# quadram-institute-bioscience/tatajuba

Measured on AMD Instinct MI355X. Metric: reads/s (whole node), 150 bp synthetic FASTQ, homopolymer scan + context histogram, higher is better.
Workload: dtype u8/u64

## Files before the change

### tatajuba_amd/csrc/hopo_device.hip

```cpp

#include <hip/hip_runtime.h>
#include <rccl/rccl.h>
#include <dlfcn.h>
#include <mutex>
#include <string>
#include <new>
#include <stdint.h>
#include <stdio.h>
#include <stdlib.h>
#include <string.h>
#include <stdarg.h>
#include <limits.h>
#include <float.h>
#include <algorithm>
#include <vector>

#include "../../include/tatajuba_amd.h"
#include "../../include/tatajuba_variants.h"
#include "../../include/tatajuba_features.h"
#include "../../include/tatajuba_effects.h"
#include "../../include/tatajuba_locate.h"

typedef unsigned long long u64;
typedef unsigned int u32;
// ... 1544 lines not shown
        }
      }
      else
      for (int cb0 = 0; cb0 < ncand; cb0 += FK_BLOCK) {
        if (!all_fit) sink.reserve1 ((u32) min (ncand - cb0, FK_BLOCK));
        if (cb0 + 64 * wave >= ncand) continue;
        const int ci = cb0 + tid;
        const bool valid = ci < ncand;
        const u32 s = T.cand[min (ci, ncand - 1)];
        const u32 q = s + 1u, u = s - vk;
        const u32 *ps = &T.st[q >> 5], *pl = &T.lt[u >> 5], *pc = &T.code[u >> 4];
        u32 s0 = ps[0], s1 = ps[1], l0 = pl[0], l1 = pl[1], w0 = pc[0], w1 = pc[1], w2 = pc[2];
        asm volatile ("" : "+v"(s0), "+v"(s1), "+v"(l0), "+v"(l1), "+v"(w0), "+v"(w1), "+v"(w2));
        const u32 len = (u32) __builtin_ctz (__builtin_amdgcn_alignbit (s1, s0, q) | 0x80000000u) + 1u;
        const u32 need = len + vk2;
        const u32 room = v32 - need;
        const u32 notl = ~__builtin_amdgcn_alignbit (l1, l0, u);
        const u32 bad = __builtin_amdgcn_bitop3_b32 (notl << (room & 31u), room >> 31, (len - (valid ? vmp : 0x1000u)) >> 31, 0xFE);
        const bool ok = bad == 0u;
        if (valid && (int) room < 0) {
          const u64 rec = fast_general_tract (T, seq, n_bytes, tile * (long) FK_OWN - FK_HL, (int) s, k, mprime, (ncand_all >= 0x40000000u));
          if (rec != 0ull) sink.store1 (atomicAdd (&sink.L.n, 1u), (u32) rec, (u32) (rec >> 32));
        }
        const u64 okm = __builtin_amdgcn_ballot_w64 (ok);
        u32 araw;
        lds_add_issue (sink.count_addr (), (u32) __builtin_popcountll (okm), araw);
        const u32 sh = u + u;
        const u32 clo = __builtin_amdgcn_alignbit (w1, w0, sh), chi = __builtin_amdgcn_alignbit (w2, w1, sh);
        const u32 l = clo & vkm;
        const u32 cb = (clo >> vk2) & 3u;
        const u32 r = (u32) ((((u64) chi << 32) | clo) >> (vk2 + len + len)) & vkm;
        u32 rcl = revcomp_v32 (l, M55, vrs), rcr = revcomp_v32 (r, M55, vrs);
        if ((ncand_all >= 0x40000000u)) {
          const u32 nb = bits32 (T.np, (int) u);
          if ((nb << ((v32 - need) & 31u)) != 0u && need <= 32u) {
            rcl = revcomp_v32 (l | (u32) spread_pairs (nb & ((1u << k) - 1u)), M55, vrs);
            rcr = revcomp_v32 (r | (u32) spread_pairs ((nb >> ((u32) k + len)) & ((1u << k) - 1u)), M55, vrs);
          }
        }
        const bool rev = cb >= 2u;
        const u32 c0 = rev ? rcr : l, c1 = rev ? rcl : r;
        const u32 fld24 = __builtin_amdgcn_perm (0u, 0x10140C08u, (cb << 24) | 0x000C0C0Cu);
        const u32 lo = c1 | (len << 24);
        const u32 hi = c0 | fld24;
        const u32 at = lds_collect (araw) + (u32) __builtin_amdgcn_mbcnt_hi ((u32) (okm >> 32), __builtin_amdgcn_mbcnt_lo ((u32) okm, 0u));
        if constexpr (LOG) sink.store1ok (ok, at, lo, hi, (u32) lane);
        else sink.store1v (ok ? at : (u32) sink.S + (u32) lane, lo, hi, vh0, vh1, vm27);
      }
    }
    lds_barrier ();
    if (nt >= grp_end) { gpar ^= 1u; grp_end = nt + FK_GROUP; }
    tile = nt;
    it++;
  }
  flush_slow ();
  sink.finish ();
}

#define PL_BLOCK 512
#define PL_WG_PER_CU 2
template <int W>
__global__ __launch_bounds__ (PL_BLOCK, PL_BLOCK * PL_WG_PER_CU / 256)
void partition_log_kernel (LogSpace LG, Buckets BK, DevCounters *ctr, int k)
{
  static_assert (W == 1 || W == 2, "the log holds one-word and two-word records");
  typedef StageLds<W, 2> Lds;
  __shared__ Lds L;
  constexpr u32 RB = TJ_LOGB / W;
  static_assert (Lds::S == (int) RB && Lds::WS == W, "one pass per log block");
  constexpr u32 RR = RB / PL_BLOCK;
  static_assert (RR % 4 == 0, "bins are kept four to a register");
  const u32 tid = threadIdx.x, lane = tid & 63u;
  const u32 wave = (u32) __builtin_amdgcn_readfirstlane ((int) (tid >> 6));
  if (tid < TJ_P) L.hist[tid] = 0;
  u32 cur_j = TJ_EMPTY, cur_chunk = TJ_NOCHUNK;
  lds_barrier ();
  const u32 n_blocks = min (*LG.next, LG.n_blocks);
  u32 b = blockIdx.x;
  if (b >= n_blocks) return;
  u64 w[RR][W];
  u32 n = min (LG.count[b], RB), nn = 0;
  auto load_block = [&] (u32 blk, u32 cnt) {
    const u64 *__restrict__ src = LG.log + ((u64) blk << TJ_LOGB_SHIFT);
    const u32 w0 = tid & ~63u;
#pragma unroll
    for (u32 r = 0; r < RR; r++) {
#pragma unroll
      for (int j = 0; j < W; j++) w[r][j] = 0;
      if (w0 + r * PL_BLOCK < cnt) {
        if constexpr (W == 1) w[r][0] = (src + r * PL_BLOCK)[tid];
        else { const ulonglong2 v = reinterpret_cast<const ulonglong2 *> (src + 2u * r * PL_BLOCK)[tid]; w[r][0] = v.x; w[r][1] = v.y; }
      }
    }
  };
  auto bucket_of = [&] (const u64 *rec) -> u32 {
    if constexpr (W == 1) return bucket_of_rec1 ((u32) rec[0], (u32) (rec[0] >> 32));
    else { u64 c0, c1; u32 base, len10, flag; unpack_raw<W> (rec, k, c0, c1, base, len10, flag); return bucket_of_key (c0, c1, base, len10); }
  };
  load_block (b, n);
  while (true) {
    const u32 bn = b + gridDim.x;
    const bool more = bn < n_blocks;
    if (more) nn = min (LG.count[bn], RB);
    u32 tq = tid;
    asm volatile ("" : "+v"(tq));
    u32 pk[RR / 4];
#pragma unroll
    for (u32 r = 0; r < RR / 4; r++) pk[r] = 0;
    if (n) {
#pragma unroll
      for (u32 r = 0; r < RR; r++) {
        const u32 bin = bucket_of (w[r]);
        pk[r >> 2] |= bin << (8u * (r & 3u));
        if (tid + r * PL_BLOCK < n) atomicAdd (&L.hist[bin], 1u);
      }
      lds_barrier ();
      if (wave < TJ_P / 64) {
        const uint4 h4 = *reinterpret_cast<const uint4 *> (&L.hist[4 * lane]);
        const u32 tot = h4.x + h4.y + h4.z + h4.w;
        const u32 e0 = wave_inclusive_scan (tot) - tot;
        if ((lane >> 4) == wave) *reinterpret_cast<uint4 *> (&L.offs[4 * lane]) = make_uint4 (e0, e0 + h4.x, e0 + h4.x + h4.y, e0 + h4.x + h4.y + h4.z);
        const u32 cnt = L.hist[tid], off = L.offs[tid];
        u64 a1 = 0, a2 = 0;
        u32 thr = off + cnt;
        if (cnt) {
          const u32 p0 = atomicAdd (&BK.cursors[tid * TJ_CSTRIDE], cnt);
          const u32 ch = (u32) TJ_CH0 << BK.ch_shift;
          bucket_claim_ahead_range (BK, tid, p0, cnt, ctr);
          const u32 j0 = chunk_of_pos (BK, p0), j1 = chunk_of_pos (BK, p0 + cnt - 1);
          if (j0 != cur_j) { cur_j = j0; cur_chunk = bucket_chunk_id (BK, tid, j0, true, ctr); }
          if (cur_chunk != TJ_NOCHUNK) a1 = (u64) (size_t) (BK.pool + ((u64) cur_chunk * ch + (p0 - j0 * ch)) * W) - (8ull * W) * off;
          if (j1 != j0) {
            thr = off + ((j0 + 1u) * ch - p0);
            cur_j = j0 + 1u; cur_chunk = bucket_chunk_id (BK, tid, j0 + 1u, true, ctr);
            if (cur_chunk != TJ_NOCHUNK) a2 = (u64) (size_t) (BK.pool + ((u64) cur_chunk * ch) * W) - (8ull * W) * thr;
          }
        }
        reinterpret_cast<uint4 *> (L.gbase)[tid] = make_uint4 ((u32) a1, (u32) (a1 >> 32) | (thr << 16), (u32) a2, (u32) (a2 >> 32));
      }
      lds_barrier ();
      if (tid < TJ_P) L.hist[tid] = 0;
#pragma unroll
      for (u32 r = 0; r < RR; r++)
        if (tid + r * PL_BLOCK < n) {
          const u32 bin = (pk[r >> 2] >> (8u * (r & 3u))) & 255u;
          const u32 d = atomicAdd (&L.offs[bin], 1u);
#pragma unroll
          for (int j = 0; j < W; j++) L.rec[d * W + j] = w[r][j];
          L.bin[d] = (unsigned char) bin;
        }
      lds_barrier ();
      for (u32 r0 = 0; r0 < RR; r0 += 4) {
        if (r0 * PL_BLOCK >= n) break;
        u32 cb[4]; uint4 e[4]; u64 cw[4][W];
#pragma unroll
        for (u32 h = 0; h < 4; h++) cb[h] = L.bin[tq + (r0 + h) * PL_BLOCK];
#pragma unroll
        for (u32 h = 0; h < 4; h++) {
          e[h] = reinterpret_cast<const uint4 *> (L.gbase)[cb[h]];
#pragma unroll
          for (int j = 0; j < W; j++) cw[h][j] = L.rec[(tq + (r0 + h) * PL_BLOCK) * W + j];
        }
#pragma unroll
        for (u32 h = 0; h < 4; h++) {
          const u32 i = tq + (r0 + h) * PL_BLOCK;
          const u64 a = (i < (e[h].y >> 16)) ? (((u64) (e[h].y & 0xFFFFu) << 32) | e[h].x) : (((u64) e[h].w << 32) | e[h].z);
          if (i < n && a != 0ull) {
            typedef __attribute__((address_space(1))) u64 *gwords_t;
            gwords_t q = (gwords_t) (a + (u64) (8u * W * i));
#pragma unroll
            for (int j = 0; j < W; j++) q[j] = cw[h][j];
          }
        }
      }
      lds_barrier ();
    }
    if (!more) break;
    load_block (bn, nn);
    n = nn; b = bn;
  }
}

template <int W>
__global__ void nrun_fixup_bins_kernel (const uint8_t *__restrict__ seq, long n_bytes, int k, int mprime,
                                        Buckets BK, DevCounters *ctr, const FixEntry *fix, u32 fix_cap, int par)
{
  nrun_fixup_entries<W> (seq, n_bytes, k, mprime, BK, ctr, fix, fix_cap, par, blockIdx.x * (u64) blockDim.x + threadIdx.x, (u64) gridDim.x * blockDim.x);
}

template <int W>
__global__ void bin_elems_kernel (const u64 *__restrict__ elems5, long n, int k, Buckets BK, DevCounters *ctr)
{
  for (long i = blockIdx.x * (long) blockDim.x + threadIdx.x; i < n; i += (long) gridDim.x * blockDim.x) {
    const u64 m = elems5[5 * i + 2];
    bucket_insert_slow<W> (elems5[5 * i], elems5[5 * i + 1], (u32) (m & 3ull), (u32) ((m >> TJ_META_LEN_SHIFT) & 0x3FFull),
                           (u32) ((m >> TJ_META_FLAG_SHIFT) & 3ull), k, BK, ctr);
  }
}

template <int W>
__global__ void unpack_buckets_kernel (Buckets BK, int k, u64 *__restrict__ out, u64 cap, u64 *n_out)
{
  const u32 b = blockIdx.x;
  const u32 n = BK.cursors[b * TJ_CSTRIDE];
  for (u32 i = threadIdx.x; i < n; i += blockDim.x) {
    u64 c0, c1; u32 base, len10, flag;
    const u64 at = bucket_slot (BK, b, i, false, nullptr);
    if (at == ~0ull) continue;
    unpack_raw<W> (BK.pool + at * W, k, c0, c1, base, len10, flag);
    if (flag == 3u) continue;
    const u64 o = atomicAdd (n_out, 1ull);
    if (o < cap) { u64 *q = out + 3 * o; q[0] = c0; q[1] = c1; q[2] = make_meta (base, len10, flag); }
  }
}

__global__ void init_table_kernel (u32 *table, u32 maxj, u32 *pool_next)
{
  const u32 b = blockIdx.x * blockDim.x + threadIdx.x;
  if (b < TJ_P) table[(u64) b * maxj] = b;
  if (b == 0) *pool_next = TJ_P;
}

__global__ void clear_buckets_kernel (u32 *cursors, DevCounters *ctr, u32 *table, u32 maxj, int ch_shift, FinCounts *fin, u32 *bins, int nbins,
                                      DevCounters *snap_ctr, u32 *snap_cursors, FinPlan *plan, u32 *__restrict__ fine = nullptr, int fine_bits = 0)
{
  const u32 b = blockIdx.x;
  if (snap_ctr) {
    if (threadIdx.x == 0) {
      snap_cursors[b] = cursors[b * TJ_CSTRIDE];
      if (b == 0) {
        snap_cursors[TJ_P] = cursors[TJ_P * TJ_CSTRIDE];
        if (plan) { plan->n1_exact = (long) fin->n_kept; plan->ovf_exact = fin->overflow; }
      }
    }
    if (b == 0) for (u32 i = threadIdx.x; i < sizeof (DevCounters) / 4; i += blockDim.x) reinterpret_cast<u32 *> (snap_ctr)[i] = reinterpret_cast<const u32 *> (ctr)[i];
    __syncthreads ();
  }
  if (b == 0) for (u32 i = threadIdx.x; i < sizeof (DevCounters) / 4; i += blockDim.x) if (i != offsetof (DevCounters, n_undefined) / 4 && i != offsetof (DevCounters, n_undefined) / 4 + 1) reinterpret_cast<u32 *> (ctr)[i] = 0;
  if (table) {
    u32 used = maxj;
    if (ch_shift >= 0) used = min (maxj, ((cursors[b * TJ_CSTRIDE] / TJ_CH0) >> ch_shift) + 3u);
    for (u32 j = threadIdx.x; j < used; j += blockDim.x) table[(u64) b * maxj + j] = j ? TJ_EMPTY : b;
  }
  if (fine) {
    const int gid = (int) (b * blockDim.x + threadIdx.x), gsz = (int) (gridDim.x * blockDim.x);
    if (plan->ok) {
      const int shift = fine_bits - plan->nbits, run = 1 << shift, nb = plan->nbins;
      for (int i = gid; i < nb; i += gsz) {
        u32 sum = 0;
        if (shift >= 2) {
          uint4 *f4 = reinterpret_cast<uint4 *> (fine) + (size_t) i * (run >> 2);
          for (int j = 0; j < (run >> 2); j++) { const uint4 v = f4[j]; sum += v.x + v.y + v.z + v.w; }
          for (int j = 0; j < (run >> 2); j++) f4[j] = make_uint4 (0, 0, 0, 0);
        }
        else {
          for (int j = 0; j < run; j++) sum += fine[(i << shift) + j];
          for (int j = 0; j < run; j++) fine[(i << shift) + j] = 0;
        }
        bins[i] = sum;
      }
    }
    else for (int i = gid; i < (1 << fine_bits); i += gsz) fine[i] = 0;
// ... 1372 lines not shown
    const u32 st = binstart[bin], s = binstart[bin + 1] - st, o0 = binout[bin];
    for (u32 t0 = 0; t0 < s; t0 += 64) {
      const u32 t = t0 + lane;
      if (t < s) {
        const long u = (long) o0 + tpos[st + t];
        if (u < cap) {
          const u64 a0 = rec[3 * (u64) (st + t)], a1 = rec[3 * (u64) (st + t) + 1], am = rec[3 * (u64) (st + t) + 2];
          const u32 tot = ttot[st + t];
          if (tot != 0xFFFFFFFFu) {
            for (int q = 0; q < n_samples; q++) counts[u * n_samples + q] = 0;
            u64 m = am & ((1ull << TJ_META_SAMPLE_SHIFT) - 1ull);
            m = (m & ~(0xFFFFFull << TJ_META_COUNT_SHIFT)) | (((u64) tot & 0xFFFFFull) << TJ_META_COUNT_SHIFT);
            m = (m & ~(7ull << TJ_META_FLAG_SHIFT)) | ((u64) ((tot >> 28) & 7u) << TJ_META_FLAG_SHIFT);
            keys[3 * u] = a0; keys[3 * u + 1] = a1; keys[3 * u + 2] = m;
          }
        }
      }
      __builtin_amdgcn_wave_barrier ();
      asm volatile ("s_waitcnt vmcnt(0)" ::: "memory");
      if (t < s) {
        const long u = (long) o0 + tpos[st + t];
        if (u < cap) {
          const u64 am = rec[3 * (u64) (st + t) + 2];
          counts[u * n_samples + (int) (am >> TJ_META_SAMPLE_SHIFT)] = meta_count (am);
        }
      }
    }
  }
}

__global__ void set_int_kernel (int *p, int v) { *p = v; }


__global__ void merge_tag_kernel (const u64 *__restrict__ in, u64 *__restrict__ out, long n, const long *__restrict__ starts, int n_samples)
{
  for (long i = blockIdx.x * (long) blockDim.x + threadIdx.x; i < n; i += (long) gridDim.x * blockDim.x) {
    int lo = 0, hi = n_samples;
    while (hi - lo > 1) { const int mid = (lo + hi) >> 1; if (starts[mid] <= i) lo = mid; else hi = mid; }
    out[3 * i] = in[3 * i]; out[3 * i + 1] = in[3 * i + 1];
    out[3 * i + 2] = (in[3 * i + 2] & ((1ull << TJ_META_SAMPLE_SHIFT) - 1ull)) | ((u64) lo << TJ_META_SAMPLE_SHIFT);
  }
}

__global__ void merge_write_kernel (const u64 *__restrict__ rec, long n, const u32 *__restrict__ flags, const u32 *__restrict__ segid,
                                    int n_samples, u64 *__restrict__ keys, int *__restrict__ counts, u32 *__restrict__ totals, u32 *__restrict__ orflags, long cap)
{
  for (long i = blockIdx.x * (long) blockDim.x + threadIdx.x; i < n; i += (long) gridDim.x * blockDim.x) {
    const u32 seg = segid[i] + flags[i] - 1u;
    if ((long) seg >= cap) continue;
    const u64 meta = rec[3 * i + 2];
    const int sample = (int) (meta >> TJ_META_SAMPLE_SHIFT);
    const int cnt = meta_count (meta);
    counts[(long) seg * n_samples + sample] = cnt;
    atomicAdd (&totals[seg], (u32) cnt);
    atomicOr (&orflags[seg], (u32) (meta >> TJ_META_FLAG_SHIFT) & 7u);
    if (flags[i]) { keys[3 * (long) seg] = rec[3 * i]; keys[3 * (long) seg + 1] = rec[3 * i + 1]; keys[3 * (long) seg + 2] = meta; }
  }
}

__global__ void merge_totals_kernel (u64 *__restrict__ keys, const u32 *__restrict__ totals, const u32 *__restrict__ orflags, const u32 *n_seg_p, long cap)
{
  const long n_seg = min ((long) *n_seg_p, cap);
  for (long j = blockIdx.x * (long) blockDim.x + threadIdx.x; j < n_seg; j += (long) gridDim.x * blockDim.x) {
    u64 m = keys[3 * j + 2] & ((1ull << TJ_META_SAMPLE_SHIFT) - 1ull);
    m = (m & ~(0xFFFFFull << TJ_META_COUNT_SHIFT)) | (((u64) totals[j] & 0xFFFFFull) << TJ_META_COUNT_SHIFT);
    m = (m & ~(7ull << TJ_META_FLAG_SHIFT)) | ((u64) (orflags[j] & 7u) << TJ_META_FLAG_SHIFT);
    keys[3 * j + 2] = m;
  }
}



struct DevBuf
{
  void *p = nullptr;
  size_t cap = 0;
};

#define TJ_SCAN_PIECE_TARGET (1ull << 30)

struct DevState { alignas (256) DevCounters ctr; alignas (256) FinCounts fin; alignas (256) u32 cursors[TJ_P + 1]; alignas (256) FinPlan plan;
                  alignas (256) DevCounters snap_ctr; alignas (256) u32 snap_cursors[TJ_P + 1]; alignas (256) u32 pad[4]; };

struct StageTimer
{
  hipEvent_t e0 = nullptr, e1 = nullptr;
  bool timed = false;
  hipError_t create () { const hipError_t e = hipEventCreate (&e0); return e != hipSuccess ? e : hipEventCreate (&e1); }
  void destroy () { if (e0) (void) hipEventDestroy (e0); if (e1) (void) hipEventDestroy (e1); }
  hipError_t begin (hipStream_t stream) { return hipEventRecord (e0, stream); }
  hipError_t end (hipStream_t stream) { return hipEventRecord (e1, stream); }
  bool elapsed (int device, float &ms) const
  { return timed && hipSetDevice (device) == hipSuccess && hipEventSynchronize (e1) == hipSuccess && hipEventElapsedTime (&ms, e0, e1) == hipSuccess; }
  double ms (int device) const { float f = 0.f; return elapsed (device, f) ? (double) f : -1.0; }
};
enum { T_SCAN, T_FIN, T_MERGE, T_TRACT, T_UNION, T_UNION_STATS, T_REF, T_LOCATE, T_LOCATED_TRACTS, T_VARIANTS, T_ANNOTATION, T_TRACT_FEATURES, T_SEED_ORDER, T_LOCATE_GAPPED, T_CODING, T_VARIANT_EFFECTS, TJ_N_TIMERS };

struct tjamd_counter
{
  int device = 0, k = 0, W = 4, n_cu = 256;
  hipStream_t own_stream = nullptr, stream = nullptr;
  DevCounters *d_ctr = nullptr, *h_ctr = nullptr;
  DevCounters *d_lctr = nullptr;
  u32 *d_cursors = nullptr, *h_cursors = nullptr;
  DevBuf pool, table, stage, fix, loc, prefix, rawlist, slow;
  DevBuf log, logmeta;
  int log_mode = 1;
  bool log_next_clean[2] = {false, false};
  hipEvent_t ev_p1 = nullptr;
#define TJ_PIECE_EVENTS 64
  hipEvent_t ev_pa[TJ_PIECE_EVENTS] = {}, ev_pb[TJ_PIECE_EVENTS] = {};
  int n_piece_ev = 0;
  StageTimer timer[TJ_N_TIMERS];
  DevBuf ts_cov, ts_aux;
  long union_cand = -1;
  DevBuf ut_tot, ut_lev, ut_fb, ut_slots;
  DevBuf lc_work;
  bool part_timed = false;
  int fast_mode = 1;
  u32 pool_chunks = 0, maxj = 0;
  int ch_shift = -1;
  u64 bucket_bound = 0;
  u64 chunk_bound = 0;
  long n_raw_known = 0;
  u64 raw_bound = 0;
  long n_undefined = 0;
  double slack = 1.0;
  DevBuf alt, hist, flags, segid, headpos, keep, outpos, scan_tmp, kept, idx_i, idx_f, cov, bins, binstart, binctx, ovf, grp_jt, grp_hist, fine;
  u32 bin_rank_max = BS_RANK_MAX;
  FinCounts *d_fin = nullptr, *h_fin = nullptr;
  struct DevState *d_state = nullptr, *h_state = nullptr;
  void *h_kept = nullptr; size_t h_kept_cap = 0;
  bool bins_zeroed = false;
  bool fine_dirty = false;
  bool bins_counted = false;
  long n_kept = 0; int n_idx = 0, coverage = 0, status = -1;
  hipEvent_t ev_done = nullptr;
  hipEvent_t ev_agg = nullptr;
  hipStream_t order_stream = nullptr;
  int fin_pending = 0;
  int fin_rb = 0, fin_mc = 0; bool fin_speculative = false, fin_plan_ahead = false; u64 fin_kept_cap = 0;
  hipEvent_t marks[8] = {nullptr, nullptr, nullptr, nullptr, nullptr, nullptr, nullptr, nullptr};
  unsigned mark_seq = 0;
  long last_scan_launches = 0;
  unsigned scan_seq = 0;
  size_t piece_target = TJ_SCAN_PIECE_TARGET;
  int scan_grid_cap = 0;
  bool buckets_clean = false;
  long plan_mismatches = 0;
  bool ctr_clean = false;
};

static int ensure (DevBuf &b, size_t bytes, hipStream_t stream, size_t keep_bytes = 0)
{
  if (bytes <= b.cap) return TJAMD_OK;
  size_t want = std::max (bytes, b.cap + b.cap / 2);
  void *np = nullptr;
  hipError_t e = hipMalloc (&np, want);
  if (e != hipSuccess && want > bytes) { want = bytes; e = hipMalloc (&np, want); }
  if (e != hipSuccess) return set_err (TJAMD_ERR_HIP, "hipMalloc of %zu bytes failed: %s", want, hipGetErrorString (e));
  if (b.p) {
    if (keep_bytes) HIPCHK (hipMemcpyAsync (np, b.p, keep_bytes, hipMemcpyDeviceToDevice, stream));
    HIPCHK (hipStreamSynchronize (stream));
    HIPCHK (hipFree (b.p));
  }
  b.p = np; b.cap = want;
  return TJAMD_OK;
}

static void release (DevBuf &b) { if (b.p) (void) hipFree (b.p); b.p = nullptr; b.cap = 0; }

extern "C" tjamd_counter *tjamd_counter_create (int device, int kmer_size)
{
  int n = tjamd_device_count ();
  if (n <= 0) { set_err (TJAMD_ERR_NO_DEVICE, "no HIP device visible: the homopolymer-tract engine needs an MI355X (no CPU fallback)"); return NULL; }
  if (device < 0 || device >= n) { set_err (TJAMD_ERR_ARG, "device %d out of range [0,%d)", device, n); return NULL; }
  if (kmer_size < 2 || kmer_size > 32) { set_err (TJAMD_ERR_ARG, "kmer_size %d outside [2,32] (reference clamp: src/main.c:184-185)", kmer_size); return NULL; }
  HIPCHK_NULL (hipSetDevice (device));
  tjamd_counter *c = new tjamd_counter ();
  c->device = device; c->k = kmer_size;
  c->W = (kmer_size <= 12) ? 1 : (kmer_size <= 28) ? 2 : 4;
  hipDeviceProp_t prop;
  HIPCHK_NULL (hipGetDeviceProperties (&prop, device));
  c->n_cu = prop.multiProcessorCount > 0 ? prop.multiProcessorCount : 256;
  const char *bm = getenv ("TATAJUBA_AMD_BIN_MAX");
  if (bm && atoi (bm) >= 1 && atoi (bm) <= BS_RANK_MAX) c->bin_rank_max = (u32) atoi (bm);
  const char *pc = getenv ("TATAJUBA_AMD_SCAN_PIECE");
  if (pc && atol (pc) >= 4096) c->piece_target = (size_t) atol (pc);
  const char *sk = getenv ("TATAJUBA_AMD_SINK");
  if (sk && !strcmp (sk, "fused")) c->log_mode = 0;
  if (sk && !strcmp (sk, "log")) c->log_mode = 2;
  const char *fm = getenv ("TATAJUBA_AMD_FAST");
  if (fm && atoi (fm) >= 0 && atoi (fm) <= 2) c->fast_mode = atoi (fm);
  const char *sg = getenv ("TATAJUBA_AMD_SCAN_GRID");
  if (sg && atoi (sg) >= 1) c->scan_grid_cap = atoi (sg);
  const char *sl = getenv ("TATAJUBA_AMD_BUCKET_SLACK");
  if (sl && atof (sl) >= 1.0) c->slack = atof (sl);
  HIPCHK_NULL (hipStreamCreateWithFlags (&c->own_stream, hipStreamNonBlocking));
  c->stream = c->own_stream;
  HIPCHK_NULL (hipMalloc ((void **) &c->d_state, sizeof (DevState)));
  HIPCHK_NULL (hipMalloc ((void **) &c->d_lctr, sizeof (DevCounters)));
  HIPCHK_NULL (hipHostMalloc ((void **) &c->h_state, sizeof (DevState), hipHostMallocDefault));
  c->d_ctr = &c->d_state->ctr; c->d_fin = &c->d_state->fin;
  HIPCHK_NULL (hipMalloc ((void **) &c->d_cursors, (size_t) (TJ_P + 1) * TJ_CSTRIDE * 4));
  HIPCHK_NULL (hipMemsetAsync (c->d_cursors, 0, (size_t) (TJ_P + 1) * TJ_CSTRIDE * 4, c->stream));
  c->h_ctr = &c->h_state->ctr; c->h_fin = &c->h_state->fin; c->h_cursors = c->h_state->cursors;
  memset (c->h_state, 0, sizeof (DevState));
  HIPCHK_NULL (hipMemsetAsync (c->d_state, 0, sizeof (DevState), c->stream));
  HIPCHK_NULL (hipMemsetAsync (c->d_lctr, 0, sizeof (DevCounters), c->stream));
  for (StageTimer &t : c->timer) HIPCHK_NULL (t.create ());
  HIPCHK_NULL (hipEventCreate (&c->ev_p1));
  HIPCHK_NULL (hipEventCreateWithFlags (&c->ev_done, hipEventDisableTiming));
  HIPCHK_NULL (hipEventCreateWithFlags (&c->ev_agg, hipEventDisableTiming));
  HIPCHK_NULL (hipStreamSynchronize (c->stream));
  return c;
}

extern "C" void tjamd_counter_destroy (tjamd_counter *c)
{
  if (!c) return;
  (void) hipSetDevice (c->device);
  (void) hipStreamSynchronize (c->stream);
  DevBuf *all[] = {&c->log, &c->logmeta, &c->pool, &c->table, &c->stage, &c->fix, &c->loc, &c->prefix, &c->rawlist, &c->slow, &c->alt, &c->hist, &c->flags, &c->segid, &c->headpos,
                   &c->keep, &c->outpos, &c->scan_tmp, &c->kept, &c->idx_i, &c->idx_f, &c->cov, &c->bins, &c->binstart, &c->binctx, &c->ovf, &c->grp_jt, &c->grp_hist, &c->fine,
                   &c->ts_cov, &c->ts_aux, &c->ut_tot, &c->ut_lev, &c->ut_fb, &c->ut_slots, &c->lc_work};
  for (DevBuf *b : all) release (*b);
  for (hipEvent_t ev : c->marks) if (ev) (void) hipEventDestroy (ev);
  if (c->d_state) (void) hipFree (c->d_state);
  if (c->d_lctr) (void) hipFree (c->d_lctr);
  if (c->d_cursors) (void) hipFree (c->d_cursors);
  if (c->h_state) (void) hipHostFree (c->h_state);
  if (c->h_kept) (void) hipHostFree (c->h_kept);
  for (StageTimer &t : c->timer) t.destroy ();
  if (c->ev_p1) (void) hipEventDestroy (c->ev_p1);
  for (int i = 0; i < TJ_PIECE_EVENTS; i++) { if (c->ev_pa[i]) (void) hipEventDestroy (c->ev_pa[i]); if (c->ev_pb[i]) (void) hipEventDestroy (c->ev_pb[i]); }
  if (c->ev_done) (void) hipEventDestroy (c->ev_done);
  if (c->ev_agg) (void) hipEventDestroy (c->ev_agg);
  if (c->own_stream) (void) hipStreamDestroy (c->own_stream);
  delete c;
}

extern "C" int tjamd_counter_device (const tjamd_counter *c) { return c ? c->device : -1; }

extern "C" int tjamd_counter_set_stream (tjamd_counter *c, void *hip_stream)
{
  if (!c) return set_err (TJAMD_ERR_ARG, "null counter");
  HIPCHK (hipSetDevice (c->device));
  HIPCHK (hipStreamSynchronize (c->stream));
  c->stream = hip_stream ? (hipStream_t) hip_stream : c->own_stream;
  return TJAMD_OK;
}

extern "C" int tjamd_counter_set_order_stream (tjamd_counter *c, void *hip_stream)
{
  if (!c) return set_err (TJAMD_ERR_ARG, "null counter");
  HIPCHK (hipSetDevice (c->device));
  HIPCHK (hipStreamSynchronize (c->stream));
  if (c->order_stream) HIPCHK (hipStreamSynchronize (c->order_stream));
  c->order_stream = (hipStream_t) hip_stream;
  return TJAMD_OK;
}

static Buckets make_buckets (const tjamd_counter *c)
{
  Buckets B;
  B.pool = (u64 *) c->pool.p; B.table = (u32 *) c->table.p; B.cursors = c->d_cursors; B.pool_next = c->d_cursors + TJ_P * TJ_CSTRIDE;
  B.pool_chunks = c->pool_chunks; B.maxj = c->maxj; B.ch_shift = (u32) std::max (c->ch_shift, 0);
  return B;
}

static int clear_buckets (tjamd_counter *c, bool snapshot = false)
{
  if (!c->buckets_clean || snapshot) {
    const bool fused = snapshot && c->fine_dirty && c->bins.p != nullptr;
    hipLaunchKernelGGL (clear_buckets_kernel, dim3 (TJ_P), dim3 (256), 0, c->stream, c->d_cursors, c->d_ctr,
                        (u32 *) (c->maxj ? c->table.p : nullptr), c->maxj, c->ch_shift, c->d_fin, (u32 *) c->bins.p, c->bins.p ? BS_MAXBINS : 0,
                        snapshot ? &c->d_state->snap_ctr : (DevCounters *) nullptr, snapshot ? c->d_state->snap_cursors : (u32 *) nullptr,
                        snapshot ? &c->d_state->plan : (FinPlan *) nullptr, fused ? (u32 *) c->fine.p : (u32 *) nullptr, fine_bin_bits (c->k));
    HIPCHK (hipGetLastError ());
    c->buckets_clean = true;
    c->ctr_clean = true;
    c->bins_zeroed = c->bins.p != nullptr && !fused;
    if (fused) { c->fine_dirty = false; c->bins_counted = true; }
  }
  c->n_raw_known = 0; c->raw_bound = 0; c->bucket_bound = 0; c->chunk_bound = TJ_P; c->ch_shift = -1;
  return TJAMD_OK;
}

extern "C" int tjamd_counter_reset (tjamd_counter *c)
{
  if (!c) return set_err (TJAMD_ERR_ARG, "null counter");
  HIPCHK (hipSetDevice (c->device));
  if (!(c->ctr_clean && c->fin_pending == 0 && c->n_undefined == 0)) HIPCHK (hipMemsetAsync (c->d_ctr, 0, sizeof (DevCounters), c->stream));
  int rc = clear_buckets (c);
// ... 174 lines not shown
  const size_t keep = std::min<size_t> (c->pool.cap, (size_t) (c->chunk_bound * ch * c->W * 8));
  rc = ensure (c->pool, (size_t) ((records / ch + 2 * TJ_P + 1) * ch * c->W * 8), c->stream, keep);
  if (rc) return rc;
  c->pool_chunks = (u32) std::min<u64> (c->pool.cap / (ch * c->W * 8), TJ_NOCHUNK - 1);
  c->buckets_clean = c->buckets_clean && c->table.p != nullptr;
  return ensure_table (c, (c->bucket_bound + records + ch - 1) / ch + 3);
}

static int scan_device_piece (tjamd_counter *c, const void *d_stream, size_t n_bytes, int min_tract_size, bool first, bool last)
{
  int rc = TJAMD_OK;
  if (n_bytes < 64 && d_stream != c->stage.p) {
    rc = ensure (c->stage, 256, c->stream);
    if (rc) return rc;
    HIPCHK (hipMemcpyAsync (c->stage.p, d_stream, n_bytes, hipMemcpyDeviceToDevice, c->stream));
    d_stream = c->stage.p;
  }
  const int mprime = std::max (min_tract_size, 2);
  const u64 bound = (u64) ((double) (n_bytes / (size_t) mprime + 1) * c->slack);
  const long n_tiles = (long) ((n_bytes + TJ_SB_TILE - 1) / TJ_SB_TILE);
  const int grid = (int) std::min<long> (n_tiles, (long) c->n_cu * TJ_SB_WG_PER_CU);
  rc = ensure_buckets (c, bound, grid + 1);
  c->raw_bound += (u64) (n_bytes / (size_t) mprime) + 1u;
  if (!rc) rc = ensure (c->fix, (size_t) TJ_FIX_CAP * sizeof (FixEntry), c->stream);
  const long n_ftiles = (long) ((n_bytes + FK_OWN - 1) / FK_OWN);
  const int fgrid = (int) std::min<long> (n_ftiles, (long) c->n_cu * FK_WG_PER_CU);
  const int lgrid = (int) std::min<long> (n_ftiles * ((FK_OWN + TJ_SB_TILE - 1) / TJ_SB_TILE), (long) c->n_cu * TJ_SB_WG_PER_CU);
  if (!rc && c->fast_mode) rc = ensure (c->slow, (size_t) n_ftiles * 4 + 64, c->stream);
  if (rc) return rc;
  const uint8_t *seq = (const uint8_t *) d_stream;
  const Buckets BK = make_buckets (c);
  FixEntry *fix = (FixEntry *) c->fix.p;
  const int par = (int) (c->scan_seq++ & 1u);
  if (first) HIPCHK (c->timer[T_SCAN].begin (c->stream));
  const TileSrc plain = {nullptr, 0};
  auto capped = [c] (long g) { return (unsigned) (c->scan_grid_cap >= 1 ? std::min<long> (g, (long) c->scan_grid_cap) : g); };
  const bool use_fast = c->fast_mode && n_bytes < ((size_t) 1 << 31) - (1u << 20);
  const bool use_log = use_fast && c->W <= c->log_mode;
  LogSpace LG = {nullptr, nullptr, nullptr, 0u};
  const int fgrid_log = (int) std::min<long> (n_ftiles, (long) c->n_cu * FK_LOG_WG_PER_CU);
  if (use_log) {
    const u64 n_blocks = ((bound * (u64) c->W) >> TJ_LOGB_SHIFT) + 3ull * (u64) fgrid_log + 8ull;
    rc = ensure (c->log, (size_t) (((n_blocks << TJ_LOGB_SHIFT) + 64ull * (u64) fgrid_log) * 8ull), c->stream);
    if (!rc && (size_t) (n_blocks + 2) * 4 > c->logmeta.cap) {
      rc = ensure (c->logmeta, (size_t) (n_blocks + 2) * 4 * 2, c->stream);
      c->log_next_clean[0] = c->log_next_clean[1] = false;
    }
    if (rc) return rc;
    u32 *meta = (u32 *) c->logmeta.p;
    if (!c->log_next_clean[par]) HIPCHK (hipMemsetAsync (meta + par, 0, 4, c->stream));
    LG.log = (u64 *) c->log.p; LG.next = meta + par; LG.next_other = meta + (par ^ 1); LG.count = meta + 2; LG.n_blocks = (u32) n_blocks;
    c->log_next_clean[par] = false; c->log_next_clean[par ^ 1] = true;
  }
  else c->log_next_clean[par ^ 1] = c->log_next_clean[par ^ 1] && true;
#define TJ_LAUNCH_SCAN(WW) do { \
    if (use_fast) { \
       \
      if (WW <= 2 && use_log) \
        hipLaunchKernelGGL ((scan_fast_kernel<(WW <= 2 ? WW : 1), true>), dim3 (capped (fgrid_log)), dim3 (FK_BLOCK), 0, c->stream, seq, (long) n_bytes, n_ftiles, c->k, mprime, BK, c->d_ctr, \
                            (u32 *) c->slow.p, par, c->fast_mode == 2 ? 1 : 0, LG); \
      else \
      hipLaunchKernelGGL (scan_fast_kernel<WW>, dim3 (capped (fgrid)), dim3 (FK_BLOCK), 0, c->stream, seq, (long) n_bytes, n_ftiles, c->k, mprime, BK, c->d_ctr, \
                          (u32 *) c->slow.p, par, c->fast_mode == 2 ? 1 : 0, LG); \
      const TileSrc listed = {(const u32 *) c->slow.p, (long) FK_OWN}; \
      hipLaunchKernelGGL (scan_bins_kernel<WW>, dim3 (capped (lgrid)), dim3 (TJ_SB_BLOCK), 0, c->stream, seq, (long) n_bytes, 0l, c->k, mprime, BK, c->d_ctr, fix, (u32) TJ_FIX_CAP, par, listed); \
    } \
    else { \
      hipLaunchKernelGGL (scan_bins_kernel<WW>, dim3 (capped (grid)), dim3 (TJ_SB_BLOCK), 0, c->stream, seq, (long) n_bytes, n_tiles, c->k, mprime, BK, c->d_ctr, fix, (u32) TJ_FIX_CAP, par, plain); \
      hipLaunchKernelGGL (nrun_fixup_bins_kernel<WW>, dim3 (64), dim3 (256), 0, c->stream, seq, (long) n_bytes, c->k, mprime, BK, c->d_ctr, (const FixEntry *) fix, (u32) TJ_FIX_CAP, par); \
    } \
  } while (0)
  switch (c->W) {
    case 1: TJ_LAUNCH_SCAN (1); break;
    case 2: TJ_LAUNCH_SCAN (2); break;
    default: TJ_LAUNCH_SCAN (4); break;
  }
#undef TJ_LAUNCH_SCAN
  HIPCHK (hipGetLastError ());
  if (last) HIPCHK (c->timer[T_SCAN].end (c->stream));
  if (first) c->n_piece_ev = 0;
  const bool mid_events = use_log && !last && c->n_piece_ev < TJ_PIECE_EVENTS;
  if (mid_events) {
    const int i = c->n_piece_ev;
    if (!c->ev_pa[i]) { HIPCHK (hipEventCreate (&c->ev_pa[i])); HIPCHK (hipEventCreate (&c->ev_pb[i])); }
    HIPCHK (hipEventRecord (c->ev_pa[i], c->stream));
  }
  if (use_log) {
    if (c->W == 1) hipLaunchKernelGGL (partition_log_kernel<1>, dim3 (capped ((long) c->n_cu * PL_WG_PER_CU)), dim3 (PL_BLOCK), 0, c->stream, LG, BK, c->d_ctr, c->k);
    else hipLaunchKernelGGL (partition_log_kernel<2>, dim3 (capped ((long) c->n_cu * PL_WG_PER_CU)), dim3 (PL_BLOCK), 0, c->stream, LG, BK, c->d_ctr, c->k);
    HIPCHK (hipGetLastError ());
  }
  if (mid_events) { HIPCHK (hipEventRecord (c->ev_pb[c->n_piece_ev], c->stream)); c->n_piece_ev++; }
  if (last) { HIPCHK (hipEventRecord (c->ev_p1, c->stream)); c->part_timed = use_log; }
  c->timer[T_SCAN].timed = true;
  c->last_scan_launches = first ? 1 : c->last_scan_launches + 1;
  c->status = -1;
  return TJAMD_OK;
}


__global__ __launch_bounds__ (1024)
void find_cut_kernel (const uint8_t *__restrict__ seq, unsigned long long first_from, unsigned long long step, unsigned long long n, unsigned long long *out)
{
  __shared__ unsigned long long best;
  const unsigned long long from = first_from + (unsigned long long) blockIdx.x * step;
  if (threadIdx.x == 0) best = ~0ull;
  __syncthreads ();
  for (unsigned long long base = from & ~15ull; base < n; base += 1024ull * 16ull) {
    const unsigned long long p = base + 16ull * threadIdx.x + 15ull;
    if (p >= from && p < n && seq[p] == (uint8_t) '\n') atomicMin (&best, p);
    __syncthreads ();
    if (best != ~0ull) break;
    __syncthreads ();
  }
  if (threadIdx.x == 0) out[blockIdx.x] = best;
}

extern "C" int tjamd_scan_device (tjamd_counter *c, const void *d_stream, size_t n_bytes, int min_tract_size)
{
  int rc = check_scan_args (c, min_tract_size);
  if (rc) return rc;
  if (n_bytes == 0) return TJAMD_OK;
  if (!d_stream || ((uintptr_t) d_stream & 15u)) return set_err (TJAMD_ERR_ARG, "device stream pointer must be non-null and 16-byte aligned");
  HIPCHK (hipSetDevice (c->device));
  const size_t piece_target = c->piece_target, piece_max = piece_target + piece_target / 2;
  if (n_bytes <= piece_max) return scan_device_piece (c, d_stream, n_bytes, min_tract_size, true, true);
  const uint8_t *seq = (const uint8_t *) d_stream;
  const size_t n_cuts = (n_bytes - 1) / piece_target;
  std::vector<unsigned long long> cuts (n_cuts);
  rc = ensure (c->prefix, 64 + 8 * n_cuts, c->stream);
  if (rc) return rc;
  hipLaunchKernelGGL (find_cut_kernel, dim3 ((unsigned) n_cuts), dim3 (1024), 0, c->stream, seq, (unsigned long long) piece_target, (unsigned long long) piece_target,
                      (unsigned long long) n_bytes, (unsigned long long *) c->prefix.p);
  HIPCHK (hipMemcpyAsync (cuts.data (), c->prefix.p, 8 * n_cuts, hipMemcpyDeviceToHost, c->stream));
  HIPCHK (hipStreamSynchronize (c->stream));
  size_t off = 0, next_cut = 0;
  bool first = true;
  while (off < n_bytes) {
    size_t end = n_bytes;
    if (n_bytes - off > piece_max) {
      while (next_cut < n_cuts && (cuts[next_cut] == ~0ull || cuts[next_cut] + 1 < off + piece_target / 2)) next_cut++;
      if (next_cut < n_cuts && cuts[next_cut] + 1 < n_bytes) end = (size_t) cuts[next_cut] + 1;
    }
    rc = scan_device_piece (c, seq + off, end - off, min_tract_size, first, end == n_bytes);
    if (rc) return rc;
    if (end < n_bytes && (rc = sync_counters (c))) return rc;
    off = end;
    first = false;
  }
  return TJAMD_OK;
}

extern "C" int tjamd_scan_host (tjamd_counter *c, const void *h_stream, size_t n_bytes, int min_tract_size)
{
  if (!c) return set_err (TJAMD_ERR_ARG, "null counter");
  if (n_bytes == 0) return TJAMD_OK;
  if (!h_stream) return set_err (TJAMD_ERR_ARG, "null host stream");
  HIPCHK (hipSetDevice (c->device));
  int rc = ensure (c->stage, (n_bytes + 255) & ~(size_t) 255, c->stream);
  if (rc) return rc;
  HIPCHK (hipMemcpyAsync (c->stage.p, h_stream, n_bytes, hipMemcpyHostToDevice, c->stream));
  return tjamd_scan_device (c, c->stage.p, n_bytes, min_tract_size);
}

extern "C" long tjamd_scan_host_located (tjamd_counter *c, const void *h_stream, size_t n_bytes, int min_tract_size,
                                          tjamd_located_record *out, long capacity)
{
// ... 3382 lines not shown
```

Measured before the change: 11.51 billion.

## Software-pipeline partition_log kernel and create timing events without system fences

Restructures the partition_log loop so the next log block's global load, histogram count and cursor reservation overlap with the scatter and global write of the current block. This cuts the barriers per iteration and hides global load and atomic latency behind LDS work. An explicit s_waitcnt asm with operand lists tied to specific RR/W values keeps the loaded registers live. Separately, the stage timer and piece events are created with hipEventDisableSystemFence to lower the cost of recording them, which may affect host visibility of timing.

After: 11.54 billion (median of 3 runs). Within noise of the previous version (+0.2%).

```diff
diff --git a/tatajuba_amd/csrc/hopo_device.hip b/tatajuba_amd/csrc/hopo_device.hip
--- a/tatajuba_amd/csrc/hopo_device.hip
+++ b/tatajuba_amd/csrc/hopo_device.hip
@@ -1650,7 +1650,7 @@
   u32 n = min (LG.count[b], RB), nn = 0;
   auto load_block = [&] (u32 blk, u32 cnt) {
     const u64 *__restrict__ src = LG.log + ((u64) blk << TJ_LOGB_SHIFT);
-    const u32 w0 = tid & ~63u;
+    const u32 w0 = wave * 64u;
 #pragma unroll
     for (u32 r = 0; r < RR; r++) {
 #pragma unroll
@@ -1665,87 +1665,119 @@
     if constexpr (W == 1) return bucket_of_rec1 ((u32) rec[0], (u32) (rec[0] >> 32));
     else { u64 c0, c1; u32 base, len10, flag; unpack_raw<W> (rec, k, c0, c1, base, len10, flag); return bucket_of_key (c0, c1, base, len10); }
   };
+  u32 pk[RR / 4];
+  auto count_sweep = [&] (u32 cnt_rec) {
+#pragma unroll
+    for (u32 r = 0; r < RR / 4; r++) pk[r] = 0;
+    if (cnt_rec == 0) return;
+#pragma unroll
+    for (u32 r = 0; r < RR; r++) {
+      const u32 bin = bucket_of (w[r]);
+      pk[r >> 2] |= bin << (8u * (r & 3u));
+      if (tid + r * PL_BLOCK < cnt_rec) atomicAdd (&L.hist[bin], 1u);
+    }
+  };
+  u32 o_cnt = 0, o_off = 0, o_p0 = 0;
+  auto owners_reserve = [&] (u32 cnt_rec) {
+    o_cnt = 0; o_off = 0; o_p0 = 0;
+    if (cnt_rec && wave < TJ_P / 64) {
+      const uint4 h4 = *reinterpret_cast<const uint4 *> (&L.hist[4 * lane]);
+      const u32 tot = h4.x + h4.y + h4.z + h4.w;
+      const u32 e0 = wave_inclusive_scan (tot) - tot;
+      if ((lane >> 4) == wave) *reinterpret_cast<uint4 *> (&L.offs[4 * lane]) = make_uint4 (e0, e0 + h4.x, e0 + h4.x + h4.y, e0 + h4.x + h4.y + h4.z);
+      o_cnt = L.hist[tid]; o_off = L.offs[tid];
+      if (o_cnt) o_p0 = atomicAdd (&BK.cursors[tid * TJ_CSTRIDE], o_cnt);
+    }
+  };
+  auto owners_place = [&] (u32 cnt_rec) {
+    if (cnt_rec && wave < TJ_P / 64) {
+      const u32 cnt = o_cnt, off = o_off, p0 = o_p0;
+      u64 a1 = 0, a2 = 0;
+      u32 thr = off + cnt;
+      if (cnt) {
+        const u32 ch = (u32) TJ_CH0 << BK.ch_shift;
+        bucket_claim_ahead_range (BK, tid, p0, cnt, ctr);
+        const u32 j0 = chunk_of_pos (BK, p0), j1 = chunk_of_pos (BK, p0 + cnt - 1);
+        if (j0 != cur_j) { cur_j = j0; cur_chunk = bucket_chunk_id (BK, tid, j0, true, ctr); }
+        if (cur_chunk != TJ_NOCHUNK) a1 = (u64) (size_t) (BK.pool + ((u64) cur_chunk * ch + (p0 - j0 * ch)) * W) - (8ull * W) * off;
+        if (j1 != j0) {
+          thr = off + ((j0 + 1u) * ch - p0);
+          cur_j = j0 + 1u; cur_chunk = bucket_chunk_id (BK, tid, j0 + 1u, true, ctr);
+          if (cur_chunk != TJ_NOCHUNK) a2 = (u64) (size_t) (BK.pool + ((u64) cur_chunk * ch) * W) - (8ull * W) * thr;
+        }
+      }
+      reinterpret_cast<uint4 *> (L.gbase)[tid] = make_uint4 ((u32) a1, (u32) (a1 >> 32) | (thr << 16), (u32) a2, (u32) (a2 >> 32));
+    }
+  };
+  auto wait_for_all = [&] () {
+    if constexpr (W == 1)
+      asm volatile ("s_waitcnt vmcnt(0)" : "+v"(o_p0), "+v"(w[0][0]), "+v"(w[1][0]), "+v"(w[2][0]), "+v"(w[3][0]), "+v"(w[4][0]), "+v"(w[5][0]), "+v"(w[6][0]), "+v"(w[7][0]),
+                    "+v"(w[8][0]), "+v"(w[9][0]), "+v"(w[10][0]), "+v"(w[11][0]), "+v"(w[12][0]), "+v"(w[13][0]), "+v"(w[14][0]), "+v"(w[15][0]) :: "memory");
+    else {
+      asm volatile ("s_waitcnt vmcnt(0)" : "+v"(o_p0), "+v"(w[0][0]), "+v"(w[1][0]), "+v"(w[2][0]), "+v"(w[3][0]), "+v"(w[4][0]), "+v"(w[5][0]), "+v"(w[6][0]), "+v"(w[7][0]) :: "memory");
+      asm volatile ("" : "+v"(w[0][W - 1]), "+v"(w[1][W - 1]), "+v"(w[2][W - 1]), "+v"(w[3][W - 1]), "+v"(w[4][W - 1]), "+v"(w[5][W - 1]), "+v"(w[6][W - 1]), "+v"(w[7][W - 1]));
+    }
+    static_assert ((W == 1 && RR == 16) || (W == 2 && RR == 8), "asm operand lists");
+  };
+  if (b + gridDim.x < n_blocks) nn = min (LG.count[b + gridDim.x], RB);
   load_block (b, n);
+  wait_for_all ();
+  count_sweep (n);
+  lds_barrier ();
+  owners_reserve (n);
+  lds_barrier ();
   while (true) {
     const u32 bn = b + gridDim.x;
     const bool more = bn < n_blocks;
-    if (more) nn = min (LG.count[bn], RB);
     u32 tq = tid;
     asm volatile ("" : "+v"(tq));
-    u32 pk[RR / 4];
-#pragma unroll
-    for (u32 r = 0; r < RR / 4; r++) pk[r] = 0;
-    if (n) {
-#pragma unroll
-      for (u32 r = 0; r < RR; r++) {
-        const u32 bin = bucket_of (w[r]);
-        pk[r >> 2] |= bin << (8u * (r & 3u));
-        if (tid + r * PL_BLOCK < n) atomicAdd (&L.hist[bin], 1u);
-      }
-      lds_barrier ();
-      if (wave < TJ_P / 64) {
-        const uint4 h4 = *reinterpret_cast<const uint4 *> (&L.hist[4 * lane]);
-        const u32 tot = h4.x + h4.y + h4.z + h4.w;
-        const u32 e0 = wave_inclusive_scan (tot) - tot;
-        if ((lane >> 4) == wave) *reinterpret_cast<uint4 *> (&L.offs[4 * lane]) = make_uint4 (e0, e0 + h4.x, e0 + h4.x + h4.y, e0 + h4.x + h4.y + h4.z);
-        const u32 cnt = L.hist[tid], off = L.offs[tid];
-        u64 a1 = 0, a2 = 0;
-        u32 thr = off + cnt;
-        if (cnt) {
-          const u32 p0 = atomicAdd (&BK.cursors[tid * TJ_CSTRIDE], cnt);
-          const u32 ch = (u32) TJ_CH0 << BK.ch_shift;
-          bucket_claim_ahead_range (BK, tid, p0, cnt, ctr);
-          const u32 j0 = chunk_of_pos (BK, p0), j1 = chunk_of_pos (BK, p0 + cnt - 1);
-          if (j0 != cur_j) { cur_j = j0; cur_chunk = bucket_chunk_id (BK, tid, j0, true, ctr); }
-          if (cur_chunk != TJ_NOCHUNK) a1 = (u64) (size_t) (BK.pool + ((u64) cur_chunk * ch + (p0 - j0 * ch)) * W) - (8ull * W) * off;
-          if (j1 != j0) {
-            thr = off + ((j0 + 1u) * ch - p0);
-            cur_j = j0 + 1u; cur_chunk = bucket_chunk_id (BK, tid, j0 + 1u, true, ctr);
-            if (cur_chunk != TJ_NOCHUNK) a2 = (u64) (size_t) (BK.pool + ((u64) cur_chunk * ch) * W) - (8ull * W) * thr;
-          }
+    if (tid < TJ_P) L.hist[tid] = 0;
+#pragma unroll
+    for (u32 r = 0; r < RR; r++)
+      if (tid + r * PL_BLOCK < n) {
+        const u32 bin = (pk[r >> 2] >> (8u * (r & 3u))) & 255u;
+        const u32 d = atomicAdd (&L.offs[bin], 1u);
+#pragma unroll
+        for (int j = 0; j < W; j++) L.rec[d * W + j] = w[r][j];
+        L.bin[d] = (unsigned char) bin;
+      }
+    if (more) load_block (bn, nn);
+    const u32 bnn = bn + gridDim.x;
+    u32 n3 = 0;
+    if (more && bnn < n_blocks) n3 = LG.count[bnn];
+    lds_barrier ();
+    wait_for_all ();
+    count_sweep (more ? nn : 0u);
+    owners_place (n);
+    lds_barrier ();
+    const u32 keep_n = n;
+    owners_reserve (more ? nn : 0u);
+#pragma unroll
+    for (u32 r0 = 0; r0 < RR; r0 += 4) if (r0 * PL_BLOCK < keep_n) {
+      u32 cb[4]; uint4 e[4]; u64 cw[4][W];
+#pragma unroll
+      for (u32 h = 0; h < 4; h++) cb[h] = L.bin[tq + (r0 + h) * PL_BLOCK];
+#pragma unroll
+      for (u32 h = 0; h < 4; h++) {
+        e[h] = reinterpret_cast<const uint4 *> (L.gbase)[cb[h]];
+#pragma unroll
+        for (int j = 0; j < W; j++) cw[h][j] = L.rec[(tq + (r0 + h) * PL_BLOCK) * W + j];
+      }
+#pragma unroll
+      for (u32 h = 0; h < 4; h++) {
+        const u32 i = tq + (r0 + h) * PL_BLOCK;
+        const u64 a = (i < (e[h].y >> 16)) ? (((u64) (e[h].y & 0xFFFFu) << 32) | e[h].x) : (((u64) e[h].w << 32) | e[h].z);
+        if (i < keep_n && a != 0ull) {
+          typedef __attribute__((address_space(1))) u64 *gwords_t;
+          gwords_t q = (gwords_t) (a + (u64) (8u * W * i));
+#pragma unroll
+          for (int j = 0; j < W; j++) q[j] = cw[h][j];
         }
-        reinterpret_cast<uint4 *> (L.gbase)[tid] = make_uint4 ((u32) a1, (u32) (a1 >> 32) | (thr << 16), (u32) a2, (u32) (a2 >> 32));
-      }
-      lds_barrier ();
-      if (tid < TJ_P) L.hist[tid] = 0;
-#pragma unroll
-      for (u32 r = 0; r < RR; r++)
-        if (tid + r * PL_BLOCK < n) {
-          const u32 bin = (pk[r >> 2] >> (8u * (r & 3u))) & 255u;
-          const u32 d = atomicAdd (&L.offs[bin], 1u);
-#pragma unroll
-          for (int j = 0; j < W; j++) L.rec[d * W + j] = w[r][j];
-          L.bin[d] = (unsigned char) bin;
-        }
-      lds_barrier ();
-      for (u32 r0 = 0; r0 < RR; r0 += 4) {
-        if (r0 * PL_BLOCK >= n) break;
-        u32 cb[4]; uint4 e[4]; u64 cw[4][W];
-#pragma unroll
-        for (u32 h = 0; h < 4; h++) cb[h] = L.bin[tq + (r0 + h) * PL_BLOCK];
-#pragma unroll
-        for (u32 h = 0; h < 4; h++) {
-          e[h] = reinterpret_cast<const uint4 *> (L.gbase)[cb[h]];
-#pragma unroll
-          for (int j = 0; j < W; j++) cw[h][j] = L.rec[(tq + (r0 + h) * PL_BLOCK) * W + j];
-        }
-#pragma unroll
-        for (u32 h = 0; h < 4; h++) {
-          const u32 i = tq + (r0 + h) * PL_BLOCK;
-          const u64 a = (i < (e[h].y >> 16)) ? (((u64) (e[h].y & 0xFFFFu) << 32) | e[h].x) : (((u64) e[h].w << 32) | e[h].z);
-          if (i < n && a != 0ull) {
-            typedef __attribute__((address_space(1))) u64 *gwords_t;
-            gwords_t q = (gwords_t) (a + (u64) (8u * W * i));
-#pragma unroll
-            for (int j = 0; j < W; j++) q[j] = cw[h][j];
-          }
-        }
-      }
-      lds_barrier ();
-    }
+      }
+    }
+    lds_barrier ();
     if (!more) break;
-    load_block (bn, nn);
-    n = nn; b = bn;
+    n = nn; b = bn; nn = min (n3, RB);
   }
 }
 
@@ -3284,11 +3316,13 @@
 struct DevState { alignas (256) DevCounters ctr; alignas (256) FinCounts fin; alignas (256) u32 cursors[TJ_P + 1]; alignas (256) FinPlan plan;
                   alignas (256) DevCounters snap_ctr; alignas (256) u32 snap_cursors[TJ_P + 1]; alignas (256) u32 pad[4]; };
 
+static hipError_t create_marker (hipEvent_t *ev) { return hipEventCreateWithFlags (ev, hipEventDisableSystemFence); }
+
 struct StageTimer
 {
   hipEvent_t e0 = nullptr, e1 = nullptr;
   bool timed = false;
-  hipError_t create () { const hipError_t e = hipEventCreate (&e0); return e != hipSuccess ? e : hipEventCreate (&e1); }
+  hipError_t create () { const hipError_t e = create_marker (&e0); return e != hipSuccess ? e : create_marker (&e1); }
   void destroy () { if (e0) (void) hipEventDestroy (e0); if (e1) (void) hipEventDestroy (e1); }
   hipError_t begin (hipStream_t stream) { return hipEventRecord (e0, stream); }
   hipError_t end (hipStream_t stream) { return hipEventRecord (e1, stream); }
@@ -3411,7 +3445,7 @@
   HIPCHK_NULL (hipMemsetAsync (c->d_state, 0, sizeof (DevState), c->stream));
   HIPCHK_NULL (hipMemsetAsync (c->d_lctr, 0, sizeof (DevCounters), c->stream));
   for (StageTimer &t : c->timer) HIPCHK_NULL (t.create ());
-  HIPCHK_NULL (hipEventCreate (&c->ev_p1));
+  HIPCHK_NULL (create_marker (&c->ev_p1));
   HIPCHK_NULL (hipEventCreateWithFlags (&c->ev_done, hipEventDisableTiming));
   HIPCHK_NULL (hipEventCreateWithFlags (&c->ev_agg, hipEventDisableTiming));
   HIPCHK_NULL (hipStreamSynchronize (c->stream));
@@ -3752,7 +3786,7 @@
   const bool mid_events = use_log && !last && c->n_piece_ev < TJ_PIECE_EVENTS;
   if (mid_events) {
     const int i = c->n_piece_ev;
-    if (!c->ev_pa[i]) { HIPCHK (hipEventCreate (&c->ev_pa[i])); HIPCHK (hipEventCreate (&c->ev_pb[i])); }
+    if (!c->ev_pa[i]) { HIPCHK (create_marker (&c->ev_pa[i])); HIPCHK (create_marker (&c->ev_pb[i])); }
     HIPCHK (hipEventRecord (c->ev_pa[i], c->stream));
   }
   if (use_log) {
```
